# by256/icsg3d

Measured on AMD Instinct MI355X. Metric: voxel-grids/s (fwd+bwd) for 32^3 U-Net+VAE at batch 32: value = U-Net train step (BASELINE configs[1]); DFC-VAE step (configs[2]) in secondary; both per batch in unet_plus_vae, higher is better.
Workload: dtype f32

## Files before the change

icsg3d_amd/csrc/common.h:

```cpp
#pragma once
#include <hip/hip_runtime.h>
#include <hip/hip_ext.h>
#include <atomic>
#include <cstdint>
#include <cstdio>
#include <string>
#include <vector>

namespace ics {

extern std::atomic<long long> g_kernel_launches;
struct LaunchTimer {
  virtual void next(hipEvent_t* start, hipEvent_t* stop) = 0;
  virtual ~LaunchTimer() = default;
};
extern thread_local LaunchTimer* tl_launch_timer;
template <typename... P, typename... A>
inline void ics_launch(void (*kernel)(P...), dim3 grid, dim3 block, size_t shmem, hipStream_t st, A&&... args) {
  static_assert(sizeof...(P) == sizeof...(A), "kernel argument count");
  if (tl_launch_timer != nullptr) {
    hipEvent_t e0 = nullptr, e1 = nullptr;
    tl_launch_timer->next(&e0, &e1);
    hipExtLaunchKernelGGL(kernel, grid, block, (std::uint32_t)shmem, st, e0, e1, 0u, static_cast<P>(args)...);
  } else {
// ... 68 lines not shown
  CF_NO_WINO = 256,
  CF_NO_WINO_WGRAD = 512,
  CF_NO_WINO64 = 1024,
  CF_NO_UP3 = 2048,
  CF_NO_THIN1_2STAGE = 4096,
  CF_NO_FAST_BNBWD = 8192,
  CF_NO_FUSED_HEAD = 16384,
  CF_NO_BWD_FOLD = 32768,
  CF_UP3_BIG_ALWAYS = 65536,
  CF_NO_WINOG = 262144,
  CF_NO_HEAD_BNFUSE = 524288,
  CF_NO_UP3N = 1 << 21,
  CF_NO_DGRAD_BNFUSE = 1 << 22,
  CF_NO_POOL_PRESUM = 1 << 23,
  CF_NO_HEAD_LABELS = 1 << 24,
  CF_ZBATCH = 1 << 20,
};
int conv_flags_from_env();

struct ConvGeom {
  int B, S, lgS;
  int Cin, Cout;
  int taps;
  int Kpad, Npad;
  int flags = 0;
};

struct BwdStat {
  const float* s = nullptr;
  const float* mean = nullptr;
  const float* rstd = nullptr;
// ... 97 lines not shown
```

icsg3d_amd/csrc/conv_igemm.hip:

```cpp
#include "common.h"

#ifndef ICS_GEMM_DEEP_FWD_MIN
#define ICS_GEMM_DEEP_FWD_MIN 1
#endif
#ifndef ICS_GEMM_DEEP_MIN
#define ICS_GEMM_DEEP_MIN 3
#endif
#ifndef ICS_GEMM_DEEP
#define ICS_GEMM_DEEP 1
#endif

#include <algorithm>
#include <type_traits>
#include <cstdlib>
#include <cstring>
#include <vector>

namespace ics {

typedef float f32x16 __attribute__((ext_vector_type(16)));
typedef float v4f __attribute__((ext_vector_type(4)));

#ifndef ICS_KLDA
#define ICS_KLDA 36
// ... 21 lines not shown
  if (getenv("ICSG3D_NO_THIN_C")) f |= CF_NO_THIN_C;
  if (getenv("ICSG3D_NO_COND_FOLD")) f |= CF_NO_COND_FOLD;
  if (getenv("ICSG3D_NO_WINO")) f |= CF_NO_WINO;
  if (getenv("ICSG3D_NO_WINO_WGRAD")) f |= CF_NO_WINO_WGRAD;
  if (getenv("ICSG3D_NO_WINO64")) f |= CF_NO_WINO64;
  if (getenv("ICSG3D_NO_UP3")) f |= CF_NO_UP3;
  if (getenv("ICSG3D_NO_THIN1_2STAGE")) f |= CF_NO_THIN1_2STAGE;
  if (getenv("ICSG3D_NO_FAST_BNBWD")) f |= CF_NO_FAST_BNBWD;
  if (getenv("ICSG3D_NO_FUSED_HEAD")) f |= CF_NO_FUSED_HEAD;
  if (getenv("ICSG3D_NO_BWD_FOLD")) f |= CF_NO_BWD_FOLD;
  if (getenv("ICSG3D_NO_WINOG")) f |= CF_NO_WINOG;
  if (getenv("ICSG3D_NO_HEAD_BNFUSE")) f |= CF_NO_HEAD_BNFUSE;
  if (getenv("ICSG3D_NO_UP3N")) f |= CF_NO_UP3N;
  if (getenv("ICSG3D_NO_DGRAD_BNFUSE")) f |= CF_NO_DGRAD_BNFUSE;
  if (getenv("ICSG3D_NO_POOL_PRESUM")) f |= CF_NO_POOL_PRESUM;
  if (getenv("ICSG3D_NO_HEAD_LABELS")) f |= CF_NO_HEAD_LABELS;
  { const char* e = getenv("ICSG3D_UP3_BIG_MIN_WG"); if (e && *e && strtoul(e, nullptr, 10) <= 1) f |= CF_UP3_BIG_ALWAYS; }
  return f;
}
struct DevOnce {
  bool done[64] = {false};
  bool need(int* dev) {
    int d = 0;
    if (hipGetDevice(&d) != hipSuccess || d < 0 || d >= 64) { *dev = -1; return true; }
    *dev = d;
    return !done[d];
  }
  void mark(int dev) { if (dev >= 0) done[dev] = true; }
};

// ... 58 lines not shown
  r.z = act_apply(fmaf(v.z, sc.z, sh.z), slope); r.w = act_apply(fmaf(v.w, sc.w, sh.w), slope);
  return r;
}
template <bool NOACT>
__device__ __forceinline__ v4f affine_only_or_act4(v4f v, v4f sc, v4f sh, float slope) {
  if (!NOACT) return affine_act4(v, sc, sh, slope);
  v4f r;
  r.x = fmaf(v.x, sc.x, sh.x); r.y = fmaf(v.y, sc.y, sh.y); r.z = fmaf(v.z, sc.z, sh.z); r.w = fmaf(v.w, sc.w, sh.w);
  return r;
}
__device__ __forceinline__ unsigned voxel_off(int b, int z, int y, int x, int S, int u, int C) {
  const int Ss = S >> u;
  return ((((unsigned)b * Ss + (z >> u)) * Ss + (y >> u)) * Ss + (x >> u)) * (unsigned)C;
}
__device__ __forceinline__ int clampi(int v, int hi) { return min(max(v, 0), hi); }

__device__ __forceinline__ ConvSrc pick_src(const ConvSrc& s0, const ConvSrc& s1, bool first) {
  ConvSrc s;
  s.p = first ? s0.p : s1.p;
  s.scale = first ? s0.scale : s1.scale;
  s.shift = first ? s0.shift : s1.shift;
  s.C = first ? s0.C : s1.C;
  s.up = first ? s0.up : s1.up;
  s.act = first ? s0.act : s1.act;
  s.bcast = first ? s0.bcast : s1.bcast;
  return s;
}

__device__ __forceinline__ float gather_scalar(const ConvSrc& s0, const ConvSrc& s1, int ci, int b,
                                               int z, int y, int x, int S) {
// ... 225 lines not shown
      const bool kvalid = tap < g.taps;
      int dz = 0, dy = 0, dx = 0;
      if (g.taps == 27) { dz = tap / 9 - 1; dy = (tap / 3) % 3 - 1; dx = tap % 3 - 1; }
#pragma unroll
      for (int r = 0; r < RS; ++r) {
        const int m = mrow_base + 8 * r;
        const RowPos rp = decode_row(m, S, lg);
        const int zz = rp.z + dz, yy = rp.y + dy, xx = rp.x + dx;
        const bool inb = kvalid && m < M && (unsigned)zz < (unsigned)S &&
                         (unsigned)yy < (unsigned)S && (unsigned)xx < (unsigned)S;
        ras[r] = inb ? gather_scalar(s0, s1, ci, rp.b, zz, yy, xx, S) : 0.f;
      }
    }
  };

  unsigned rowG0[RA], rowG1[RA];
  if (VEC) {
#pragma unroll
    for (int r = 0; r < RA; ++r) {
      const unsigned mc = (unsigned)min(mrow_base + 32 * r, M - 1);
      rowG0[r] = (mc * (unsigned)s0.C + (unsigned)(t & 7) * 4u) * 4u;
      rowG1[r] = (mc * (unsigned)s1.C + (unsigned)(t & 7) * 4u) * 4u;
    }
  }
  auto load_chunk_gemm = [&](int c) {
    load_b(c * 8);
    const int ci0 = c << 5;
    const bool first = ci0 < s0.C;
    const int cbase = first ? ci0 : ci0 - s0.C;
    const char* sp = reinterpret_cast<const char*>(first ? s0.p : s1.p) + (size_t)cbase * 4;
    const float slope = first ? slope0 : slope1;
    v4f sc = v4f{1.f, 1.f, 1.f, 1.f}, sh = v4f{0.f, 0.f, 0.f, 0.f};
    if (AFF) {
      sc = *reinterpret_cast<const v4f*>((first ? s0.scale : s1.scale) + cbase + (t & 7) * 4);
      sh = *reinterpret_cast<const v4f*>((first ? s0.shift : s1.shift) + cbase + (t & 7) * 4);
    }
#pragma unroll
    for (int r = 0; r < RA; ++r) {
      v4f v = *reinterpret_cast<const v4f*>(sp + (first ? rowG0[r] : rowG1[r]));
      if (AFF) v = affine_only_or_act4<NOACT>(v, sc, sh, slope);
      ra4[r] = v;
    }
  };
  auto store_a_chunk = [&]() {
// ... 150 lines not shown
  const bool gemm = VEC && !THIN && !PAR && !UP && ABL == 0 && g.taps == 1;
  if (cb < ce && gemm) {
    auto compute_g = [&](int buf) { compute_at(As + (wm * TM * 32 + li) * kLDA + lh * 4, 32, buf); };
    load_chunk_gemm(cb);
    store_b(cb & 1);
    store_a_chunk();
    __syncthreads();
#if ICS_GEMM_DEEP
    if (!AFF && TM * TN >= ICS_GEMM_DEEP_FWD_MIN) {
      v4f raA[RA], rbA[NB], raB[RA], rbB[NB];
      auto load_set = [&](int c, v4f (&xa)[RA], v4f (&xb)[NB]) {
        const char* wrow = reinterpret_cast<const char*>(wp) + (size_t)(c * 8) * (size_t)g.Npad * 16;
#pragma unroll
        for (int r = 0; r < NB; ++r) xb[r] = *reinterpret_cast<const v4f*>(wrow + bofs[r]);
        const int ci0 = c << 5;
        const bool first = ci0 < s0.C;
        const char* sp = reinterpret_cast<const char*>(first ? s0.p : s1.p) + (size_t)(first ? ci0 : ci0 - s0.C) * 4;
#pragma unroll
        for (int r = 0; r < RA; ++r) xa[r] = *reinterpret_cast<const v4f*>(sp + (first ? rowG0[r] : rowG1[r]));
      };
      auto store_set = [&](int buf, const v4f (&xa)[RA], const v4f (&xb)[NB]) {
        float* Bw = Bs + buf * B_FLOATS;
#pragma unroll
        for (int r = 0; r < NB; ++r) *reinterpret_cast<v4f*>(Bw + (t + 256 * r) * 4) = xb[r];
        __syncthreads();
#pragma unroll
        for (int r = 0; r < RA; ++r) *reinterpret_cast<v4f*>(As + ((t >> 3) + 32 * r) * kLDA + (t & 7) * 4) = xa[r];
        __syncthreads();
      };
      const int lastc = ce - 1;
      if (cb + 1 < ce) load_set(cb + 1, raA, rbA);
      int c = cb;
// ... 1064 lines not shown
    return launch_conv_fwd_thin_c(st, g, src[0], g.Cin, g.Cin, wp, bias, out, ldo, pre_act, stat_partial,
                                  rows_per_block);
  ConvSrc s0 = src[0], s1 = src[nsrc > 1 ? 1 : 0];
  if (nsrc == 1) s1.C = 0;
  const bool aff = s0.scale != nullptr || (nsrc > 1 && s1.scale != nullptr);
  const bool up = s0.up || (nsrc > 1 && s1.up);
  const int variant = up ? 2 : (aff ? 1 : 0);
  const bool noact = aff && (s0.scale == nullptr || s0.act == ACT_NONE) &&
                     (nsrc < 2 || s1.scale == nullptr || s1.act == ACT_NONE);
  ICS_TRY(fix_src(s0));
  ICS_TRY(fix_src(s1));
  bool vec = fwd_is_vec(g, s0, s1);
  const bool thin = conv_is_thin(g, s0, nsrc);
  ICS_CHECK(((size_t)g.B << (3 * g.lgS)) * (size_t)std::max(s0.C, s1.C) * 4 <= 0xffffffffull,
            "conv source larger than 4 GiB");
  const bool no_reuse = (g.flags & CF_NO_REUSE) != 0;
  const bool fold = bwd != nullptr && bwd->partial != nullptr && ksplit == 1 && vec && !thin && variant == 0 &&
                    bias == nullptr && stat_partial == nullptr && !accumulate;
  int bm, bn;
  pick_fwd_tile(g, &bm, &bn);
#define ICS_FWD_ARGS st, g, s0, s1, wp, bias, out, ldo, pre_act, stat_partial, rows_per_block, accumulate, ksplit, bwd
#define ICS_FWD(WM, WN, TM, TN)                                                                 \
  do {                                                                                          \
    if (thin) return launch_fwd_cfg<WM, WN, TM, TN, true, 0, true, true, true>(ICS_FWD_ARGS);   \
    if (!vec) return launch_fwd_cfg<WM, WN, TM, TN, false, 0, true, true>(ICS_FWD_ARGS);        \
    if (g.taps == 27 && g.S >= 4 && g.S <= (WM) * (TM) * 32 && !no_reuse) {                      \
      if (variant == 0 && fold)                                                                 \
        return launch_fwd_cfg<WM, WN, TM, TN, true, 0, false, false, false, true, false, false, true>(ICS_FWD_ARGS); \
      if (variant == 0) return launch_fwd_cfg<WM, WN, TM, TN, true, 0, false, false, false, true>(ICS_FWD_ARGS); \
      if (variant == 1 && noact)                                                                \
// ... 208 lines not shown
      sc = *reinterpret_cast<const v4f*>(sv.scale + cl0);
      sh = *reinterpret_cast<const v4f*>(sv.shift + cl0);
    }
  }
  int s_tap = 0, s_ci = 0; bool s_kvalid = false; int sdz = 0, sdy = 0, sdx = 0;
  if (!VEC) {
    const int kf = k0 + (t & 31);
    s_tap = kf / g.Cin; s_ci = kf - s_tap * g.Cin; s_kvalid = kf < K;
    if (g.taps == 27) { sdz = s_tap / 9 - 1; sdy = (s_tap / 3) % 3 - 1; sdx = s_tap % 3 - 1; }
  }

  v4f ra[VEC ? APASS : 1];
  float ras[4];
  v4f rd[DPASS];

  auto load_chunk = [&](int c) {
    const int mbase = m_begin + (c << 5);
    if (VEC) {
      const int Sh = S >> 1;
#pragma unroll
      for (int p = 0; p < APASS; ++p) {
        const int m = mbase + (t + 256 * p) / AF4;
        const int x = m & (S - 1), y = (m >> lg) & (S - 1), z = (m >> (2 * lg)) & (S - 1);
        const bool inb = kvalid && m < m_end && x != xbad && y != ybad && z != zbad;
        int idx = m + sdelta;
        if (UP) {
          const int b = m >> (3 * lg);
          const int idx_up = ((b * Sh + ((z + tdz) >> 1)) * Sh + ((y + tdy) >> 1)) * Sh + ((x + tdx) >> 1);
          idx = su ? idx_up : idx;
        }
// ... 4 lines not shown
      }
    } else {
#pragma unroll
      for (int p = 0; p < 4; ++p) {
        const int m = mbase + (t >> 5) + 8 * p;
        float v = 0.f;
        if (s_kvalid && m < m_end) {
          const RowPos r = decode_row(m, S, lg);
          const int zz = r.z + sdz, yy = r.y + sdy, xx = r.x + sdx;
          if ((unsigned)zz < (unsigned)S && (unsigned)yy < (unsigned)S && (unsigned)xx < (unsigned)S)
            v = gather_scalar(s0, s1, s_ci, r.b, zz, yy, xx, S);
        }
        ras[p] = v;
      }
    }
#pragma unroll
    for (int p = 0; p < DPASS; ++p) {
      const int idx = t + 256 * p;
      const int m = mbase + idx / DF4;
      const int n = n0 + (idx % DF4) * 4;
      const float* q = dy + (size_t)min(m, M - 1) * ldy;
      v4f v;
      if (DYVEC) {
        v = *reinterpret_cast<const v4f*>(q + min(n, n_load - 4));
        if (!(m < m_end && n < n_load)) v = v4f{0.f, 0.f, 0.f, 0.f};
      } else {
        v.x = q[min(n + 0, n_load - 1)]; v.y = q[min(n + 1, n_load - 1)];
        v.z = q[min(n + 2, n_load - 1)]; v.w = q[min(n + 3, n_load - 1)];
        const bool rowok = m < m_end;
        v.x = (rowok && n + 0 < n_load) ? v.x : 0.f; v.y = (rowok && n + 1 < n_load) ? v.y : 0.f;
        v.z = (rowok && n + 2 < n_load) ? v.z : 0.f; v.w = (rowok && n + 3 < n_load) ? v.w : 0.f;
      }
      rd[p] = v;
    }
  };
  const bool gemm = VEC && DYVEC && !UP && !THIN && ABL == 0 && g.taps == 1 && (M & 31) == 0 &&
                    (rows_per_split & 31) == 0 && n0 + NT <= n_load;
  const bool noact_g = slope == 1.f;
  unsigned aoffg[VEC ? APASS : 1], doffg[DPASS];
  if (VEC) {
#pragma unroll
    for (int p = 0; p < APASS; ++p) aoffg[p] = (unsigned)(((t + 256 * p) / AF4) * sC + cl0) * 4u;
  }
#pragma unroll
  for (int p = 0; p < DPASS; ++p) {
    const int idx = t + 256 * p;
    doffg[p] = (unsigned)((idx / DF4) * ldy + n0 + (idx % DF4) * 4) * 4u;
  }
  auto load_chunk_gemm = [&](int c, auto noact_tag) {
    constexpr bool NA = decltype(noact_tag)::value;
    const int mbase = m_begin + (c << 5);
    const char* abase = reinterpret_cast<const char*>(sp) + (size_t)mbase * (size_t)sC * 4;
    const char* dbase = reinterpret_cast<const char*>(dy) + (size_t)mbase * (size_t)ldy * 4;
    if (VEC) {
#pragma unroll
      for (int p = 0; p < APASS; ++p) {
        v4f v = *reinterpret_cast<const v4f*>(abase + aoffg[p]);
        if (AFF) v = affine_only_or_act4<NA>(v, sc, sh, slope);
        ra[p] = v;
      }
    }
#pragma unroll
    for (int p = 0; p < DPASS; ++p) rd[p] = *reinterpret_cast<const v4f*>(dbase + doffg[p]);
  };
  auto store_chunk = [&](int buf) {
    float* A = As + buf * A_FLOATS;
    float* D = Ds + buf * D_FLOATS;
    if (VEC) {
// ... 56 lines not shown
        for (int j = 0; j < TN; ++j) b[j] = D[s * 2 * NT + j * 32];
      }
#pragma unroll
      for (int i = 0; i < TM; ++i)
#pragma unroll
        for (int j = 0; j < TN; ++j)
          acc[i][j] = __builtin_amdgcn_mfma_f32_32x32x2f32(a[i], b[j], acc[i][j], 0, 0, 0);
    }
  };
#if ICS_GEMM_DEEP
  if (gemm && VEC && TM * TN >= ICS_GEMM_DEEP_MIN) {
    v4f raA[APASS], rdA[DPASS], raB[APASS], rdB[DPASS];
    auto loadS = [&](int c, v4f (&xa)[APASS], v4f (&xd)[DPASS]) {
      const int mbase = m_begin + (c << 5);
      const char* abase = reinterpret_cast<const char*>(sp) + (size_t)mbase * (size_t)sC * 4;
      const char* dbase = reinterpret_cast<const char*>(dy) + (size_t)mbase * (size_t)ldy * 4;
#pragma unroll
      for (int p = 0; p < APASS; ++p) xa[p] = *reinterpret_cast<const v4f*>(abase + aoffg[p]);
#pragma unroll
      for (int p = 0; p < DPASS; ++p) xd[p] = *reinterpret_cast<const v4f*>(dbase + doffg[p]);
    };
    auto storeS = [&](int buf, const v4f (&xa)[APASS], const v4f (&xd)[DPASS]) {
      float* A = As + buf * A_FLOATS;
      float* D = Ds + buf * D_FLOATS;
#pragma unroll
      for (int p = 0; p < APASS; ++p) {
        const int idx = t + 256 * p;
        v4f v = xa[p];
        if (AFF) v = noact_g ? affine_only_or_act4<true>(v, sc, sh, slope) : affine_only_or_act4<false>(v, sc, sh, slope);
        *reinterpret_cast<v4f*>(A + (idx / AF4) * KT + (idx % AF4) * 4) = v;
      }
// ... 623 lines not shown
#undef ICS_TNW
      ICS_HIP(hipGetLastError());
    }
    if (phase != 1)
      ICS_TRY(launch_reduce_splits(st, workspace, (M + rows - 1) / rows, n_el, g.Cout, dw, ldw, sub_rows, row_pitch,
                                   row_off));
    return 0;
  }
  ConvSrc s0 = src[0], s1 = src[nsrc > 1 ? 1 : 0];
  if (nsrc == 1) s1.C = 0;
  ICS_TRY(fix_src(s0));
  ICS_TRY(fix_src(s1));
  WgradPlan p = plan_wgrad(g, s0, nsrc, s1);
  const size_t n_elems = (size_t)g.taps * g.Cin * g.Cout;
  const int n_load4 = (g.Cout + 3) / 4 * 4;
  const bool dy_vec = (ldy % 4 == 0) && ((reinterpret_cast<uintptr_t>(dy) & 15) == 0) && (n_load4 <= ldy);
  const int n_load = dy_vec ? n_load4 : g.Cout;
  if (!dy_vec) {
    p.nt = (p.kt == 128) ? 32 : (p.kt == 64) ? 64 : 128;
    p.ntiles = (g.Npad + p.nt - 1) / p.nt;
  }
  const bool aff = src[0].scale != nullptr || (nsrc > 1 && src[1].scale != nullptr);
  const bool up = src[0].up || (nsrc > 1 && src[1].up);
  if (dy_vec && wgrad3_ok(g, s0, nsrc, s1)) {
    const Wgrad3Plan q = plan_wgrad3(g);
    ICS_CHECK((size_t)q.ksplit * n_elems <= workspace_floats, "wgrad workspace too small");
    const int arows = 32 + std::max(32 >> g.lgS, 1) + 1;
    const size_t lds = (size_t)(2 * (arows * 64 + 32 * 128) + 128) * sizeof(float);
    const dim3 grid(9 * q.cgroups * q.ntiles * q.ksplit);
    const int M3 = g.B << (3 * g.lgS);
    const bool fast = !up && g.lgS >= 4 && g.lgS <= 6 && M3 % 32 == 0 && n_load == g.Cout &&
// ... 444 lines not shown
```

icsg3d_amd/csrc/elementwise.h:

```cpp
#pragma once
#include "common.h"

#include <rccl/rccl.h>

namespace ics {

struct BnParams {
  const float* gamma;
  const float* beta;
  float* moving_mean;
  float* moving_var;
  float* mean;
  float* rstd;
  float* scale;
  float* shift;
  float* xs = nullptr;
};

struct BnSync {
  ncclComm_t comm;
  int nranks;
  double* local;
  double* gathered;
};
// ... 92 lines not shown
                    const float* cond, int ncond, int B, float* z, float* zc);
int launch_vae_loss(hipStream_t st, const float* mulv, int ld, int latent, int B, const double* mse_partial,
                    int n_mse, double n_elems, const double* pm_partial, const PmSums& pmc, float alpha, float beta,
                    float* metrics, double* sums = nullptr, int phase = 0);
int launch_vae_dz(hipStream_t st, const float* mulv, int ld, int latent, int B, const float* eps,
                  const float* dzc, int ldzc, float beta, float* dmulv);
int launch_cond_bias_table(hipStream_t st, const float* w, const float* bias, const float* cond, int C, int ncond,
                           int Cin_tot, int Cout, int B, float* T);
size_t cond_wgrad_workspace_doubles(int B, int Cout);
int launch_cond_wgrad(hipStream_t st, const float* dy, int B, int S, int Cout, const float* cond, int C0, int nfold,
                      int ncond, int Cin_tot, float* dw, double* ws, size_t ws_doubles);
int launch_relu_bwd(hipStream_t st, const float* a, float* g, size_t n);
int launch_colsum_small(hipStream_t st, const float* a, int rows, int cols, int ld, float* out);
int launch_axpy(hipStream_t st, float* y, const float* x, size_t n, float a);
int launch_pool27(hipStream_t st, const float* dy, int B, int S, int N, float* out, int ldo);
int launch_permute_up_dw(hipStream_t st, const float* tmp, int Cu, int N, int Cin, int c_off, float* dw);

}
```

icsg3d_amd/csrc/elementwise.hip:

```cpp
#include "common.h"
#include "elementwise.h"

namespace ics {

__device__ __forceinline__ double wave_sum_d(double v) {
#pragma unroll
  for (int o = 32; o > 0; o >>= 1) v += __shfl_xor(v, o);
  return v;
}
__device__ __forceinline__ float wave_sum_f(float v) {
#pragma unroll
  for (int o = 32; o > 0; o >>= 1) v += __shfl_xor(v, o);
  return v;
}
__device__ __forceinline__ float wave_max_f(float v) {
#pragma unroll
  for (int o = 32; o > 0; o >>= 1) v = fmaxf(v, __shfl_xor(v, o));
  return v;
}
__device__ __forceinline__ double block_sum_d(double v, double* sh ) {
  v = wave_sum_d(v);
  __syncthreads();
  if ((threadIdx.x & 63) == 0) sh[threadIdx.x >> 6] = v;
  __syncthreads();
// ... 1741 lines not shown
        if (sz <= 1) o[2 * 9 + dyi * 3 + dx] += P[dyi][dx];
        if (sz >= 1 && sz <= 2) o[1 * 9 + dyi * 3 + dx] += P[dyi][dx];
        if (sz >= 2) o[0 * 9 + dyi * 3 + dx] += P[dyi][dx];
      }
  }
#pragma unroll
  for (int k = 0; k < 27; ++k) *reinterpret_cast<pf4*>(out + vl * ldo + (size_t)k * N + n) = o[k];
}
int launch_pool27(hipStream_t st, const float* dy, int B, int S, int N, float* out, int ldo) {
  ICS_CHECK(N % 4 == 0 && ldo % 4 == 0, "pool27: channel counts must be multiples of 4");
  const size_t total = (size_t)B * (S / 2) * (S / 2) * (S / 2) * (N / 4);
  ICS_LAUNCH(pool27_kernel, dim3((unsigned)((total + 255) / 256)), dim3(256), 0, st, dy, B, S, N, total, out, ldo);
  ICS_HIP(hipGetLastError());
  return 0;
}
__global__ void permute_up_dw_kernel(const float* __restrict__ tmp, int Cu, int N, int Cin, int c_off,
                                     size_t total, float* __restrict__ dw) {
  const size_t i = (size_t)blockIdx.x * blockDim.x + threadIdx.x;
  if (i >= total) return;
  const int n = (int)(i % N);
  size_t r = i / N;
  const int c = (int)(r % Cu);
  const int tap = (int)(r / Cu);
  dw[((size_t)tap * Cin + c_off + c) * N + n] = tmp[(size_t)c * 27 * N + (size_t)tap * N + n];
}
int launch_permute_up_dw(hipStream_t st, const float* tmp, int Cu, int N, int Cin, int c_off, float* dw) {
  const size_t total = (size_t)27 * Cu * N;
  ICS_LAUNCH(permute_up_dw_kernel, dim3((unsigned)((total + 255) / 256)), dim3(256), 0, st, tmp, Cu, N, Cin,
                     c_off, total, dw);
  ICS_HIP(hipGetLastError());
// ... 324 lines not shown
```

icsg3d_amd/csrc/engine.hip:

```cpp
#include "common.h"
#include "elementwise.h"
#include "segment.h"
#include "scratch.h"
#include "voxelise.h"
#include "latent.h"
#include "tsne.h"
#include "render.h"
#include "monitor.h"
#include "../../include/icsg3d.h"

#include <rccl/rccl.h>
#include <roctracer/roctx.h>

#include <cmath>
#include <cstring>
#include <map>
#include <memory>
#include <mutex>
#include <vector>

namespace ics {

struct Range {
  explicit Range(const char* name) { roctxRangePushA(name); }
// ... 130 lines not shown
  ConvLayer* skip_prod = nullptr;
  ConvLayer* deferred_skip = nullptr;
  float* pooled = nullptr;
  unsigned char* pool_idx = nullptr;
  ConvSrc src[2];
  int nsrc = 1;
  bool split_up = false;
  bool wf_stale = false;
  int Cs = 0, Cu = 0;
  float *wf_skip = nullptr, *w_up = nullptr;
  float *wp_skip = nullptr, *wp_par = nullptr;
  float* w_up3 = nullptr;
  float* w_up3n = nullptr;
  float *dyS = nullptr;
  int ldS = 0;
  float *dA_skip = nullptr, *dxl = nullptr;
  float *dw_up = nullptr;
};

struct Net {
  int kind = 0;
  int device = 0;
  int flags = 0;
  hipStream_t st = nullptr;
  hipStream_t st2 = nullptr;
  hipEvent_t ev_fork = nullptr, ev_join = nullptr;
  bool side_on = true, side_dirty = false;
  bool pm_side = false;
  int maxB = 0, d = 0, C = 0;
  std::vector<void*> allocs;
// ... 257 lines not shown
}

static ConvSrc src_plain(const float* p, int C) { return ConvSrc{p, nullptr, nullptr, C, 0, ACT_NONE, 0}; }
static ConvSrc src_layer(const ConvLayer& L, int up) {
  if (L.has_bn) return ConvSrc{L.s, L.scale, L.shift, L.Cout, up, L.post_act, 0};
  return ConvSrc{L.s, nullptr, nullptr, L.Cout, up, ACT_NONE, 0};
}

static ConvGeom geom_fwd(const ConvLayer& L, int B) {
  return ConvGeom{B, L.S, ilog2(L.S), L.CinG, L.Cout, L.taps, L.Kpad, L.Npad, L.flags};
}
static ConvGeom geom_bwd(const ConvLayer& L, int B) {
  return ConvGeom{B, L.S, ilog2(L.S), L.Cout, L.CinG, L.taps, L.Kpad_b, L.Npad_b, L.flags};
}

static ConvGeom geom_up_wgrad(const ConvLayer& L, int B) {
  return ConvGeom{B, L.S / 2, ilog2(L.S / 2), L.Cu, 27 * L.Cout, 1, round_up(L.Cu, 32), L.ldS, L.flags};
}
static ConvGeom geom_up_dgrad(const ConvLayer& L, int B) {
  return ConvGeom{B, L.S / 2, ilog2(L.S / 2), L.ldS, L.Cu, 1, L.ldS, round_up(L.Cu, 32), L.flags};
}
static ConvGeom geom_skip_wgrad(const ConvLayer& L, int B) {
  return ConvGeom{B, L.S, ilog2(L.S), L.Cs, L.Cout, L.taps, round_up(L.taps * L.Cs, 32), L.Npad, L.flags};
}
static ConvGeom geom_skip_dgrad(const ConvLayer& L, int B) {
  return ConvGeom{B, L.S, ilog2(L.S), L.Cout, L.Cs, L.taps, L.Kpad_b, round_up(L.Cs, 32), L.flags};
}
static ConvGeom geom_skip_fwd(const ConvLayer& L, int B) {
  return ConvGeom{B, L.S, ilog2(L.S), L.Cs, L.Cout, L.taps, round_up(L.taps * L.Cs, 32), L.Npad, L.flags};
}
static ConvGeom geom_par_fwd(const ConvLayer& L, int B) {
  return ConvGeom{B, L.S / 2, ilog2(L.S / 2), L.Cu, L.Cout, 8, 8 * L.Cu, L.Npad, L.flags};
}
static ConvSrc src_lowres(const ConvLayer& L) { ConvSrc u = L.src[L.nsrc - 1]; u.up = 0; return u; }

static int enable_split_up(Net& n, ConvLayer& L) {
  if (n.flags & CF_NO_UPSPLIT) return 0;
  const ConvSrc& up = L.src[L.nsrc - 1];
  const int Cs = L.nsrc == 2 ? L.src[0].C : 0;
  if (!up.up || (L.nsrc == 2 && L.src[0].up) || L.taps != 27 || L.S < 2 || L.CinG != L.Cin || Cs % 32 || up.C % 32 ||
      up.bcast || L.Cout % 4)
    return 0;
  L.split_up = true;
  L.Cs = Cs; L.Cu = up.C;
  L.ldS = round_up(27 * L.Cout, 32);
  const size_t M = n.rows(L, n.maxB);
  ICS_TRY(n.alloc(&L.w_up, (size_t)L.ldS * round_up(L.Cu, 32)));
  ICS_TRY(n.alloc(&L.dyS, M / 8 * L.ldS));
  ICS_HIP(hipMemsetAsync(L.dyS, 0, M / 8 * L.ldS * sizeof(float), n.st));
  ICS_TRY(n.alloc(&L.dxl, M / 8 * L.Cu));
  ICS_TRY(n.alloc(&L.dw_up, (size_t)L.Cu * 27 * L.Cout));
  if (conv_up3_ok(geom_par_fwd(L, n.maxB), src_lowres(L)))
    ICS_TRY(n.alloc(&L.w_up3, conv_up3_weight_floats(L.Cu, L.Cout)));
  else if (L.Cs == 0 && conv_up3n_ok(geom_par_fwd(L, n.maxB), src_lowres(L)))
    ICS_TRY(n.alloc(&L.w_up3n, conv_up3n_weight_floats(L.Cu, L.Cout)));
  else
    ICS_TRY(n.alloc(&L.wp_par, (size_t)8 * 8 * L.Cu * L.Npad));
  if (L.Cs) {
    ICS_TRY(n.alloc(&L.wf_skip, (size_t)L.Kpad_b * round_up(L.Cs, 32)));
    ICS_TRY(n.alloc(&L.dA_skip, M * L.Cs));
    ICS_TRY(n.alloc(&L.wp_skip, (size_t)round_up(L.taps * L.Cs, 32) * L.Npad));
  }
  return 0;
}
// ... 47 lines not shown
static int alloc_workspaces(Net& n, bool need_bwd) {
  size_t stat = 0, bwd = 0, wg = 0, fw = 0;
  for (int b = 1; b <= n.maxB; ++b)
  for (auto& Lp : n.layers) {
    ConvLayer& L = *Lp;
    const size_t M = n.rows(L, b);
    const ConvGeom g = geom_fwd(L, b);
    const int rpb = std::min(conv_fwd_rows_per_block(g), 64);
    stat = std::max(stat, (M + rpb - 1) / rpb * 3 * (size_t)L.Npad);
    if (L.split_up) stat = std::max(stat, 8 * ((M / 8 + 63) / 64) * 3 * (size_t)L.Npad);
    fw = std::max(fw, conv_fwd_workspace_floats(g, L.src, L.nsrc));
    if (need_bwd) {
      const ConvSrc sdy = src_plain(L.dy, L.Cout);
      fw = std::max(fw, conv_fwd_workspace_floats(geom_bwd(L, b), &sdy, 1));
      if (L.split_up) {
        const ConvSrc sd = src_plain(L.dyS, L.ldS);
        fw = std::max(fw, conv_fwd_workspace_floats(geom_up_dgrad(L, b), &sd, 1));
        if (L.Cs) fw = std::max(fw, conv_fwd_workspace_floats(geom_skip_dgrad(L, b), &sdy, 1));
      }
      LayerBwd lb{};
      lb.B = b; lb.S = L.S; lb.lgS = ilog2(L.S); lb.C = L.Cout;
      if (&L != n.head) bwd = std::max(bwd, layer_bwd_workspace_floats(lb));
      wg = std::max(wg, conv_wgrad_workspace_floats(g, L.src, L.nsrc));
      if (L.wino_w)
        wg = std::max(wg, conv_wino_wgrad_workspace_floats(L.split_up ? geom_skip_wgrad(L, b) : g));
      if ((L.Cin == 1 || L.cond_fold) && (L.Cout == 16 || L.Cout == 32))
        wg = std::max(wg, conv_thin_c_wgrad_workspace_floats(g));
      if (L.split_up) {
        const ConvSrc lo = src_lowres(L);
        wg = std::max(wg, conv_wgrad_workspace_floats(geom_up_wgrad(L, b), &lo, 1));
        if (L.Cs) wg = std::max(wg, conv_wgrad_workspace_floats(geom_skip_wgrad(L, b), L.src, 1));
// ... 247 lines not shown
      L.src[0].act != ACT_NONE || !n.want_wgrad_inputs || P->tie_batch != B)
    return false;
  if (!L.wino_w || !L.wwb || L.wwb_layout != 1) return false;
  if (n.rows(L, B) * (size_t)P->Cout * sizeof(float) < 2 * n.bnfuse_min_bytes) return false;
  const ConvGeom gw = geom_skip_wgrad(L, B), gd = geom_skip_dgrad(L, B);
  const ConvSrc sdy = src_plain(L.dy, L.Cout);
  return conv_bnfuse_ok(L.S, L.Cs, L.Cout) && conv_wino_wgrad_ok(gw, L.src, 1) && conv_wino_ok(gd, &sdy, 1) &&
         conv_bnfuse_partial_floats(B, L.S, L.Cout) <= n.ws_cls_n && L.Cs % 4 == 0 &&
         pool_bnfuse_partial_doubles(n.rows(L, B) / 8, P->Cout) <= n.ws_pool_n;
}
static int conv_grads_split_up(Net& n, ConvLayer& L, int B, ConvLayer* next) {
  const size_t M = n.rows(L, B);
  const double fl_skip = 2.0 * M * 27 * L.Cs * L.Cout, fl_up = 2.0 * (M / 8) * 27 * L.Cu * L.Cout;
  const bool skipfuse = skip_bnfuse_ok(n, L, B);
  ConvLayer* P = L.skip_prod;
  n.prof.begin(n.st, "pool27:" + L.name, 0, 4.0 * M * L.Cout * (1 + 27.0 / 8));
  ICS_TRY(launch_pool27(n.st, L.dy, B, L.S, L.Cout, L.dyS, L.ldS));
  n.prof.end(n.st);
  hipStream_t ws = side_begin(n);
  if (L.Cs) {
    const ConvGeom g = geom_skip_wgrad(L, B);
    n.prof.begin(ws, "conv_wgrad:" + L.name + ".skip|", fl_skip,
                 4.0 * (M * L.Cs + M * L.Cout + 27.0 * L.Cs * L.Cout));
    const bool wino = L.wino_w && conv_wino_wgrad_ok(g, L.src, 1);
    ConvSrc sx = L.src[0];
    if (skipfuse) { sx.scale = P->xs; sx.shift = P->xs + P->Cout; }
    if (wino)
      ICS_TRY(launch_conv_wgrad_wino(ws, g, sx, L.dy, L.Cout, n.tg(L.t_w), L.Cout, n.ws_wgrad, n.ws_wgrad_n,
                                     L.Cs, L.Cin, 0, 1));
    else
    ICS_TRY(launch_conv_wgrad(ws, g, L.src, 1, L.dy, L.Cout, n.tg(L.t_w), L.Cout, n.ws_wgrad, n.ws_wgrad_n, L.Cs,
                              L.Cin, 0, 1));
    n.prof.end(ws);
// ... 8 lines not shown
    if (skipfuse) {
      const bool pend = L.db_blocks > 0;
      n.prof.begin(ws, "bnfuse:" + L.name + ".skip", 0, 0);
      ICS_TRY(launch_conv_bnfuse(ws, L.dy, B, L.S, L.Cs, L.Cin, L.Cout, pend ? L.db_partial : n.tg(L.t_b), pend ? L.db_blocks : 1,
                                 n.tp(L.t_w), n.tg(L.t_w), n.tp(P->t_gamma), n.tp(P->t_beta), P->mean, P->rstd, P->scale,
                                 nullptr, nullptr, nullptr, nullptr, n.ws_cls, n.ws_cls_n, n.ws_R, P->bn_sums));
      n.prof.end(ws);
      P->deferred_skip = &L;
    }
  }
  {
    const ConvGeom g = geom_up_wgrad(L, B);
    const ConvSrc lo = src_lowres(L);
    n.prof.begin(ws, "conv_wgrad:" + L.name + ".up|", fl_up,
                 4.0 * (M / 8 * L.Cu + M / 8 * 27.0 * L.Cout + 27.0 * L.Cu * L.Cout));
    ICS_TRY(launch_conv_wgrad(ws, g, &lo, 1, L.dyS, L.ldS, L.dw_up, 27 * L.Cout, n.ws_wgrad, n.ws_wgrad_n, 0, 0, 0, 1));
    n.prof.end(ws);
    n.prof.begin(ws, "wgrad_reduce_splits", 0, 0);
    ICS_TRY(launch_conv_wgrad(ws, g, &lo, 1, L.dyS, L.ldS, L.dw_up, 27 * L.Cout, n.ws_wgrad, n.ws_wgrad_n, 0, 0, 0, 2));
    ICS_TRY(launch_permute_up_dw(ws, L.dw_up, L.Cu, L.Cout, L.Cin, L.Cs, n.tg(L.t_w)));
    n.prof.end(ws);
  }
  if (L.Cs && !skipfuse) {
    const ConvGeom g = geom_skip_dgrad(L, B);
    ConvSrc sdy = src_plain(L.dy, L.Cout);
    n.prof.begin(n.st, "conv_dgrad:" + L.name + ".skip|", fl_skip,
                 4.0 * (M * L.Cs + M * L.Cout + 27.0 * L.Cs * L.Cout));
    if (L.wwb && conv_wino_ok(g, &sdy, 1))
      ICS_TRY(launch_conv_fwd_wino(n.st, g, sdy, L.wwb, nullptr, L.dA_skip, L.Cs, ACT_NONE, nullptr, nullptr, 0,
                                   L.wwb_layout));
    else
    ICS_TRY(launch_conv_fwd(n.st, g, &sdy, 1, L.wf_skip, nullptr, L.dA_skip, L.Cs, ACT_NONE, nullptr, nullptr, 0,
                            n.fws(), n.ws_fwd_n));
    n.prof.end(n.st);
  }
  {
    const ConvGeom g = geom_up_dgrad(L, B);
    ConvSrc sd = src_plain(L.dyS, L.ldS);
    n.prof.begin(n.st, "conv_dgrad:" + L.name + ".up|", fl_up,
                 4.0 * (M / 8 * L.Cu + M / 8 * 27.0 * L.Cout + 27.0 * L.Cu * L.Cout));
    const BwdStat bs = bwd_stat_for(n, next, B);
    int blocks = 0;
    ICS_TRY(launch_conv_fwd(n.st, g, &sd, 1, L.w_up, nullptr, L.dxl, L.Cu, ACT_NONE, nullptr, nullptr, 0, n.fws(),
                            n.ws_fwd_n, &bs, &blocks));
    bwd_stat_done(next, bs, blocks, g.Npad);
    n.prof.end(n.st);
  }
  return 0;
}

static int colsum_push(Net& n, const float* partial, int nblk, int C, float* out);
static bool dgrad_bnfuse_ok(const Net& n, const ConvLayer& L, const ConvLayer* next, int B, bool need_dA, bool param_grads) {
  if (next == nullptr || !need_dA || !param_grads || (n.flags & CF_NO_DGRAD_BNFUSE) || n.sync() != nullptr || n.side_on)
// ... 2111 lines not shown
        for (int z = 0; z < h; ++z)
          for (int y = 0; y < h; ++y)
            for (int x = 0; x < h; ++x) {
              float* o = s.dx + ((((size_t)b * h + z) * h + y) * h + x) * s.C;
              for (int c = 0; c < s.C; ++c) o[c] = 0.f;
              for (int k = 0; k < 8; ++k) {
                const size_t m = (((size_t)b * S + 2 * z + (k >> 2)) * S + 2 * y + ((k >> 1) & 1)) * S + 2 * x + (k & 1);
                for (int c = 0; c < s.C; ++c) o[c] += hA[m * ld + c0 + c];
              }
            }
    }
  }
  if (a->kernels && a->kernels_cap > 0) {
    std::string txt;
    for (const auto& r : n.prof.rows)
      if (r.label.find('|') != std::string::npos) txt += r.label + "\n";
    std::strncpy(a->kernels, txt.c_str(), (size_t)a->kernels_cap - 1);
    a->kernels[a->kernels_cap - 1] = 0;
  }
  if (n.canary_on) {
    std::string msg;
    const int bad = n.canaries_dirty(&msg);
    ICS_CHECK(bad == 0, op + "guard bytes written behind " + std::to_string(bad) + " buffer(s): " + msg);
  }
  return 0;
}

int ics_op_conv_link(ics_conv_link* a) {
  const std::string op = "ics_op_conv_link: ";
  ICS_CHECK(a != nullptr, op + "null argument");
  ICS_CHECK(a->link >= ICS_LINK_SAME && a->link <= ICS_LINK_POOL_SKIP, op + "unknown link");
// ... 309 lines not shown
```

icsg3d_amd/engine.py:

```python
from __future__ import annotations

import ctypes as C

import numpy as np

from . import _lib as L


def _f32(a):
    return np.ascontiguousarray(a, dtype=np.float32)


def _jobs4(jobs):
    jobs = np.ascontiguousarray(jobs, np.int32)
    if jobs.ndim != 2 or jobs.shape[1] != 4:
        raise ValueError("jobs must be (B, 4) int32 {structure, r0, r1, r2}, got %s" % (jobs.shape,))
    return jobs


class _Net:

    def __init__(self):
        self._h = L._H(None)
        self._lib = L.load()
# ... 538 lines not shown
            setattr(a, k, L.fptr(r[k]))
    if dout is not None:
        r["dw"], r["dbias"] = out(w.shape), out((Cout,))
        a.dw, a.dbias = L.fptr(r["dw"]), L.fptr(r["dbias"])
        if has_bn:
            r["dgamma"], r["dbeta"] = out((Cout,)), out((Cout,))
            a.dgamma, a.dbeta = L.fptr(r["dgamma"]), L.fptr(r["dbeta"])
        r["dx"] = dxs
    text = C.create_string_buffer(16384)
    a.kernels, a.kernels_cap = C.cast(text, C.c_void_p), len(text)
    L.check(lib.ics_op_conv_layer(C.byref(a)))
    if has_bn:
        r["rows_per_block"], r["blocks"] = a.rows_per_block, a.blocks
    lines = text.value.decode().splitlines()
    r["kernels"] = {k: [ln for ln in lines if ln.startswith("conv_%s:" % k)] for k in ("fwd", "dgrad", "wgrad")}
    return r


LINKS = ("same", "up", "pool", "pool_skip")


def conv_link(link, x0, layers, dout, form="unet", q=None, dout_l=None, pool_ties_all=True, max_batch=None):
    lib = L.load()
    a = L.ConvLinkArgs()
    keep = []

    def f(v):
        if v is None:
            return None
        v = _f32(v)
# ... 65 lines not shown
```

Measured before the change: 1147.

## Replace 27-tap pooled up-split operand with 8-phase pooled volume and gathered addressing

The backward of split upsampling layers used to build a pooled operand with 27 tap slabs per low-res voxel (pool27). It now builds a smaller 8-phase pooled volume on a padded (S/2+1)^3 grid (pool8). The implicit-GEMM dgrad and wgrad kernels address it through a new CF_GATHER8 mode that maps each tap to a phase and row offset. This reduces the bytes written and read for the pooled dy, at the cost of extra index arithmetic in the inner load loops and less regular access.

```diff
diff --git a/icsg3d_amd/csrc/common.h b/icsg3d_amd/csrc/common.h
--- a/icsg3d_amd/csrc/common.h
+++ b/icsg3d_amd/csrc/common.h
@@ -106,7 +106,9 @@
   CF_NO_DGRAD_BNFUSE = 1 << 22,
   CF_NO_POOL_PRESUM = 1 << 23,
   CF_NO_HEAD_LABELS = 1 << 24,
+  CF_NO_POOL8 = 1 << 25,
   CF_ZBATCH = 1 << 20,
+  CF_GATHER8 = 1 << 26,
 };
 int conv_flags_from_env();
 
diff --git a/icsg3d_amd/csrc/conv_igemm.hip b/icsg3d_amd/csrc/conv_igemm.hip
--- a/icsg3d_amd/csrc/conv_igemm.hip
+++ b/icsg3d_amd/csrc/conv_igemm.hip
@@ -59,6 +59,7 @@
   if (getenv("ICSG3D_NO_UP3N")) f |= CF_NO_UP3N;
   if (getenv("ICSG3D_NO_DGRAD_BNFUSE")) f |= CF_NO_DGRAD_BNFUSE;
   if (getenv("ICSG3D_NO_POOL_PRESUM")) f |= CF_NO_POOL_PRESUM;
+  if (getenv("ICSG3D_NO_POOL8")) f |= CF_NO_POOL8;
   if (getenv("ICSG3D_NO_HEAD_LABELS")) f |= CF_NO_HEAD_LABELS;
   { const char* e = getenv("ICSG3D_UP3_BIG_MIN_WG"); if (e && *e && strtoul(e, nullptr, 10) <= 1) f |= CF_UP3_BIG_ALWAYS; }
   return f;
@@ -147,6 +148,21 @@
   return ((((unsigned)b * Ss + (z >> u)) * Ss + (y >> u)) * Ss + (x >> u)) * (unsigned)C;
 }
 __device__ __forceinline__ int clampi(int v, int hi) { return min(max(v, 0), hi); }
+
+__device__ __forceinline__ int rowq_lin(int m, int S, int lg) {
+  const int P = S + 1;
+  const int x = m & (S - 1), y = (m >> lg) & (S - 1), z = (m >> (2 * lg)) & (S - 1), b = m >> (3 * lg);
+  return ((b * P + z) * P + y) * P + x;
+}
+__device__ __forceinline__ unsigned gather8_rcp(int N) { return 0xffffffffu / (unsigned)N + 1u; }
+__device__ __forceinline__ unsigned gather8_off(int k, int N, unsigned rcpN, int S, int ld) {
+  const int P = S + 1;
+  const int tap = (int)__umulhi((unsigned)k, rcpN), n = k - tap * N;
+  const int kz = tap / 9, ky = (tap / 3) % 3, kx = tap % 3;
+  const int roff = (((kz != 2) * P + (ky != 2)) * P + (kx != 2));
+  const int ph = 4 * (kz != 1) + 2 * (ky != 1) + (kx != 1);
+  return (unsigned)(roff * ld + ph * N + n);
+}
 
 __device__ __forceinline__ ConvSrc pick_src(const ConvSrc& s0, const ConvSrc& s1, bool first) {
   ConvSrc s;
@@ -402,11 +418,15 @@
     }
   };
 
+  const bool g8 = (g.flags & CF_GATHER8) != 0;
+  const int g8N = g8 ? g.Cin / 27 : 2;
+  const unsigned g8R = gather8_rcp(g8N);
   unsigned rowG0[RA], rowG1[RA];
   if (VEC) {
 #pragma unroll
     for (int r = 0; r < RA; ++r) {
-      const unsigned mc = (unsigned)min(mrow_base + 32 * r, M - 1);
+      unsigned mc = (unsigned)min(mrow_base + 32 * r, M - 1);
+      if (g8) mc = (unsigned)rowq_lin((int)mc, S, lg);
       rowG0[r] = (mc * (unsigned)s0.C + (unsigned)(t & 7) * 4u) * 4u;
       rowG1[r] = (mc * (unsigned)s1.C + (unsigned)(t & 7) * 4u) * 4u;
     }
@@ -414,8 +434,8 @@
   auto load_chunk_gemm = [&](int c) {
     load_b(c * 8);
     const int ci0 = c << 5;
-    const bool first = ci0 < s0.C;
-    const int cbase = first ? ci0 : ci0 - s0.C;
+    const bool first = g8 || ci0 < s0.C;
+    const int cbase = g8 ? (int)gather8_off(ci0, g8N, g8R, S, s0.C) : (first ? ci0 : ci0 - s0.C);
     const char* sp = reinterpret_cast<const char*>(first ? s0.p : s1.p) + (size_t)cbase * 4;
     const float slope = first ? slope0 : slope1;
     v4f sc = v4f{1.f, 1.f, 1.f, 1.f}, sh = v4f{0.f, 0.f, 0.f, 0.f};
@@ -596,8 +616,9 @@
 #pragma unroll
         for (int r = 0; r < NB; ++r) xb[r] = *reinterpret_cast<const v4f*>(wrow + bofs[r]);
         const int ci0 = c << 5;
-        const bool first = ci0 < s0.C;
-        const char* sp = reinterpret_cast<const char*>(first ? s0.p : s1.p) + (size_t)(first ? ci0 : ci0 - s0.C) * 4;
+        const bool first = g8 || ci0 < s0.C;
+        const int cbase = g8 ? (int)gather8_off(ci0, g8N, g8R, S, s0.C) : (first ? ci0 : ci0 - s0.C);
+        const char* sp = reinterpret_cast<const char*>(first ? s0.p : s1.p) + (size_t)cbase * 4;
 #pragma unroll
         for (int r = 0; r < RA; ++r) xa[r] = *reinterpret_cast<const v4f*>(sp + (first ? rowG0[r] : rowG1[r]));
       };
@@ -1692,6 +1713,13 @@
   const bool thin = conv_is_thin(g, s0, nsrc);
   ICS_CHECK(((size_t)g.B << (3 * g.lgS)) * (size_t)std::max(s0.C, s1.C) * 4 <= 0xffffffffull,
             "conv source larger than 4 GiB");
+  if (g.flags & CF_GATHER8) {
+    const size_t P = (size_t)g.S + 1;
+    ICS_CHECK(g.taps == 1 && nsrc == 1 && vec && !thin && variant == 0 && g.Cin % (27 * 32) == 0 && g.Kpad == g.Cin &&
+                  src[0].C >= 8 * (g.Cin / 27),
+              "gathered up-split operand: plain source, 27 tap slabs of N % 32 == 0 columns");
+    ICS_CHECK((size_t)g.B * P * P * P * (size_t)s0.C * 4 <= 0xffffffffull, "phase volumes larger than 4 GiB");
+  }
   const bool no_reuse = (g.flags & CF_NO_REUSE) != 0;
   const bool fold = bwd != nullptr && bwd->partial != nullptr && ksplit == 1 && vec && !thin && variant == 0 &&
                     bias == nullptr && stat_partial == nullptr && !accumulate;
@@ -1930,6 +1958,14 @@
   float ras[4];
   v4f rd[DPASS];
 
+  const bool g8 = DYVEC && (g.flags & CF_GATHER8) != 0;
+  unsigned gq[DPASS];
+#pragma unroll
+  for (int p = 0; p < DPASS; ++p) {
+    const int nc = max(min(n0 + ((t + 256 * p) % DF4) * 4, n_load - 4), 0);
+    gq[p] = g8 ? gather8_off(nc, g.Cout / 27, gather8_rcp(g.Cout / 27), S, ldy) : 0u;
+  }
+
   auto load_chunk = [&](int c) {
     const int mbase = m_begin + (c << 5);
     if (VEC) {
@@ -1964,25 +2000,30 @@
         ras[p] = v;
       }
     }
-#pragma unroll
-    for (int p = 0; p < DPASS; ++p) {
-      const int idx = t + 256 * p;
-      const int m = mbase + idx / DF4;
-      const int n = n0 + (idx % DF4) * 4;
-      const float* q = dy + (size_t)min(m, M - 1) * ldy;
-      v4f v;
-      if (DYVEC) {
-        v = *reinterpret_cast<const v4f*>(q + min(n, n_load - 4));
-        if (!(m < m_end && n < n_load)) v = v4f{0.f, 0.f, 0.f, 0.f};
-      } else {
-        v.x = q[min(n + 0, n_load - 1)]; v.y = q[min(n + 1, n_load - 1)];
-        v.z = q[min(n + 2, n_load - 1)]; v.w = q[min(n + 3, n_load - 1)];
-        const bool rowok = m < m_end;
-        v.x = (rowok && n + 0 < n_load) ? v.x : 0.f; v.y = (rowok && n + 1 < n_load) ? v.y : 0.f;
-        v.z = (rowok && n + 2 < n_load) ? v.z : 0.f; v.w = (rowok && n + 3 < n_load) ? v.w : 0.f;
-      }
-      rd[p] = v;
-    }
+    auto load_d = [&](auto gather_tag) {
+      constexpr bool G8 = decltype(gather_tag)::value;
+#pragma unroll
+      for (int p = 0; p < DPASS; ++p) {
+        const int idx = t + 256 * p;
+        const int m = mbase + idx / DF4;
+        const int n = n0 + (idx % DF4) * 4;
+        const int mc = min(m, M - 1);
+        const float* q = dy + (size_t)(G8 ? rowq_lin(mc, S, lg) : mc) * ldy;
+        v4f v;
+        if (DYVEC) {
+          v = *reinterpret_cast<const v4f*>(q + (G8 ? (int)gq[p] : min(n, n_load - 4)));
+          if (!(m < m_end && n < n_load)) v = v4f{0.f, 0.f, 0.f, 0.f};
+        } else {
+          v.x = q[min(n + 0, n_load - 1)]; v.y = q[min(n + 1, n_load - 1)];
+          v.z = q[min(n + 2, n_load - 1)]; v.w = q[min(n + 3, n_load - 1)];
+          const bool rowok = m < m_end;
+          v.x = (rowok && n + 0 < n_load) ? v.x : 0.f; v.y = (rowok && n + 1 < n_load) ? v.y : 0.f;
+          v.z = (rowok && n + 2 < n_load) ? v.z : 0.f; v.w = (rowok && n + 3 < n_load) ? v.w : 0.f;
+        }
+        rd[p] = v;
+      }
+    };
+    if (g8) load_d(std::true_type{}); else load_d(std::false_type{});
   };
   const bool gemm = VEC && DYVEC && !UP && !THIN && ABL == 0 && g.taps == 1 && (M & 31) == 0 &&
                     (rows_per_split & 31) == 0 && n0 + NT <= n_load;
@@ -1995,13 +2036,14 @@
 #pragma unroll
   for (int p = 0; p < DPASS; ++p) {
     const int idx = t + 256 * p;
-    doffg[p] = (unsigned)((idx / DF4) * ldy + n0 + (idx % DF4) * 4) * 4u;
+    doffg[p] = g8 ? (unsigned)(rowq_lin(idx / DF4, S, lg) * ldy + (int)gq[p]) * 4u
+                  : (unsigned)((idx / DF4) * ldy + n0 + (idx % DF4) * 4) * 4u;
   }
   auto load_chunk_gemm = [&](int c, auto noact_tag) {
     constexpr bool NA = decltype(noact_tag)::value;
     const int mbase = m_begin + (c << 5);
     const char* abase = reinterpret_cast<const char*>(sp) + (size_t)mbase * (size_t)sC * 4;
-    const char* dbase = reinterpret_cast<const char*>(dy) + (size_t)mbase * (size_t)ldy * 4;
+    const char* dbase = reinterpret_cast<const char*>(dy) + (size_t)(g8 ? rowq_lin(mbase, S, lg) : mbase) * (size_t)ldy * 4;
     if (VEC) {
 #pragma unroll
       for (int p = 0; p < APASS; ++p) {
@@ -2088,7 +2130,7 @@
     auto loadS = [&](int c, v4f (&xa)[APASS], v4f (&xd)[DPASS]) {
       const int mbase = m_begin + (c << 5);
       const char* abase = reinterpret_cast<const char*>(sp) + (size_t)mbase * (size_t)sC * 4;
-      const char* dbase = reinterpret_cast<const char*>(dy) + (size_t)mbase * (size_t)ldy * 4;
+      const char* dbase = reinterpret_cast<const char*>(dy) + (size_t)(g8 ? rowq_lin(mbase, S, lg) : mbase) * (size_t)ldy * 4;
 #pragma unroll
       for (int p = 0; p < APASS; ++p) xa[p] = *reinterpret_cast<const v4f*>(abase + aoffg[p]);
 #pragma unroll
@@ -2742,7 +2784,15 @@
   WgradPlan p = plan_wgrad(g, s0, nsrc, s1);
   const size_t n_elems = (size_t)g.taps * g.Cin * g.Cout;
   const int n_load4 = (g.Cout + 3) / 4 * 4;
-  const bool dy_vec = (ldy % 4 == 0) && ((reinterpret_cast<uintptr_t>(dy) & 15) == 0) && (n_load4 <= ldy);
+  const bool gather8 = (g.flags & CF_GATHER8) != 0;
+  if (gather8) {
+    const size_t P = (size_t)g.S + 1;
+    ICS_CHECK(g.taps == 1 && g.Cout % (27 * 4) == 0 && ldy >= 8 * (g.Cout / 27) && ldy % 4 == 0 &&
+                  (reinterpret_cast<uintptr_t>(dy) & 15) == 0 && !wgrad3_ok(g, s0, nsrc, s1),
+              "gathered up-split operand: 27 tap slabs of N % 4 == 0 columns");
+    ICS_CHECK((size_t)g.B * P * P * P * (size_t)ldy * 4 <= 0xffffffffull, "phase volumes larger than 4 GiB");
+  }
+  const bool dy_vec = (ldy % 4 == 0) && ((reinterpret_cast<uintptr_t>(dy) & 15) == 0) && (gather8 || n_load4 <= ldy);
   const int n_load = dy_vec ? n_load4 : g.Cout;
   if (!dy_vec) {
     p.nt = (p.kt == 128) ? 32 : (p.kt == 64) ? 64 : 128;
diff --git a/icsg3d_amd/csrc/elementwise.h b/icsg3d_amd/csrc/elementwise.h
--- a/icsg3d_amd/csrc/elementwise.h
+++ b/icsg3d_amd/csrc/elementwise.h
@@ -130,6 +130,7 @@
 int launch_colsum_small(hipStream_t st, const float* a, int rows, int cols, int ld, float* out);
 int launch_axpy(hipStream_t st, float* y, const float* x, size_t n, float a);
 int launch_pool27(hipStream_t st, const float* dy, int B, int S, int N, float* out, int ldo);
+int launch_pool8(hipStream_t st, const float* dy, int B, int S, int N, float* out, int ldo);
 int launch_permute_up_dw(hipStream_t st, const float* tmp, int Cu, int N, int Cin, int c_off, float* dw);
 
 }
diff --git a/icsg3d_amd/csrc/elementwise.hip b/icsg3d_amd/csrc/elementwise.hip
--- a/icsg3d_amd/csrc/elementwise.hip
+++ b/icsg3d_amd/csrc/elementwise.hip
@@ -1779,6 +1779,60 @@
   ICS_HIP(hipGetLastError());
   return 0;
 }
+__global__ __launch_bounds__(256) void pool8_kernel(const float* __restrict__ dy, int B, int S, int N, size_t total,
+                                                    float* __restrict__ out, int ldo) {
+  const size_t i = (size_t)blockIdx.x * blockDim.x + threadIdx.x;
+  if (i >= total) return;
+  const int P = (S >> 1) + 1, N4 = N >> 2;
+  const int n = (int)(i % N4) * 4;
+  const size_t row = i / N4;
+  const int ix = row % P; size_t r = row / P;
+  const int iy = r % P; r /= P;
+  const int iz = r % P;
+  const int b = (int)(r / P);
+  const pf4 zero = pf4{0.f, 0.f, 0.f, 0.f};
+  pf4 o[8];
+#pragma unroll
+  for (int k = 0; k < 8; ++k) o[k] = zero;
+#pragma unroll
+  for (int sz = 0; sz < 3; ++sz) {
+    const int z = 2 * iz - 2 + sz;
+    if ((unsigned)z >= (unsigned)S) continue;
+    pf4 lx[3][2];
+#pragma unroll
+    for (int sy = 0; sy < 3; ++sy) {
+      const int y = 2 * iy - 2 + sy;
+      pf4 v[3];
+#pragma unroll
+      for (int sx = 0; sx < 3; ++sx) {
+        const int x = 2 * ix - 2 + sx;
+        const bool ok = (unsigned)y < (unsigned)S && (unsigned)x < (unsigned)S;
+        v[sx] = ok ? *reinterpret_cast<const pf4*>(dy + ((((size_t)b * S + z) * S + y) * S + x) * N + n) : zero;
+      }
+      lx[sy][0] = v[0] + v[1];
+      lx[sy][1] = v[1] + v[2];
+    }
+#pragma unroll
+    for (int oy = 0; oy < 2; ++oy)
+#pragma unroll
+      for (int ox = 0; ox < 2; ++ox) {
+        const pf4 p = lx[oy][ox] + lx[oy + 1][ox];
+        if (sz <= 1) o[2 * oy + ox] += p;
+        if (sz >= 1) o[4 + 2 * oy + ox] += p;
+      }
+  }
+#pragma unroll
+  for (int k = 0; k < 8; ++k) *reinterpret_cast<pf4*>(out + row * ldo + (size_t)k * N + n) = o[k];
+}
+int launch_pool8(hipStream_t st, const float* dy, int B, int S, int N, float* out, int ldo) {
+  ICS_CHECK(N % 4 == 0 && ldo % 4 == 0 && ldo >= 8 * N, "pool8: channel counts must be multiples of 4");
+  const size_t P = (size_t)S / 2 + 1;
+  const size_t total = (size_t)B * P * P * P * (N / 4);
+  ICS_CHECK((total + 255) / 256 <= 0x7fffffffull, "pool8: grid too large");
+  ICS_LAUNCH(pool8_kernel, dim3((unsigned)((total + 255) / 256)), dim3(256), 0, st, dy, B, S, N, total, out, ldo);
+  ICS_HIP(hipGetLastError());
+  return 0;
+}
 __global__ void permute_up_dw_kernel(const float* __restrict__ tmp, int Cu, int N, int Cin, int c_off,
                                      size_t total, float* __restrict__ dw) {
   const size_t i = (size_t)blockIdx.x * blockDim.x + threadIdx.x;
diff --git a/icsg3d_amd/csrc/engine.hip b/icsg3d_amd/csrc/engine.hip
--- a/icsg3d_amd/csrc/engine.hip
+++ b/icsg3d_amd/csrc/engine.hip
@@ -168,6 +168,9 @@
   float* w_up3n = nullptr;
   float *dyS = nullptr;
   int ldS = 0;
+  bool pool8 = false;
+  float* Q = nullptr;
+  int ldQ = 0;
   float *dA_skip = nullptr, *dxl = nullptr;
   float *dw_up = nullptr;
 };
@@ -455,12 +458,14 @@
   return ConvGeom{B, L.S, ilog2(L.S), L.Cout, L.CinG, L.taps, L.Kpad_b, L.Npad_b, L.flags};
 }
 
+static int up_flags(const ConvLayer& L) { return L.pool8 ? (L.flags | CF_GATHER8) : L.flags; }
 static ConvGeom geom_up_wgrad(const ConvLayer& L, int B) {
-  return ConvGeom{B, L.S / 2, ilog2(L.S / 2), L.Cu, 27 * L.Cout, 1, round_up(L.Cu, 32), L.ldS, L.flags};
+  return ConvGeom{B, L.S / 2, ilog2(L.S / 2), L.Cu, 27 * L.Cout, 1, round_up(L.Cu, 32), L.ldS, up_flags(L)};
 }
 static ConvGeom geom_up_dgrad(const ConvLayer& L, int B) {
-  return ConvGeom{B, L.S / 2, ilog2(L.S / 2), L.ldS, L.Cu, 1, L.ldS, round_up(L.Cu, 32), L.flags};
-}
+  return ConvGeom{B, L.S / 2, ilog2(L.S / 2), L.ldS, L.Cu, 1, L.ldS, round_up(L.Cu, 32), up_flags(L)};
+}
+static ConvSrc src_up_pooled(const ConvLayer& L) { return L.pool8 ? src_plain(L.Q, L.ldQ) : src_plain(L.dyS, L.ldS); }
 static ConvGeom geom_skip_wgrad(const ConvLayer& L, int B) {
   return ConvGeom{B, L.S, ilog2(L.S), L.Cs, L.Cout, L.taps, round_up(L.taps * L.Cs, 32), L.Npad, L.flags};
 }
@@ -487,8 +492,16 @@
   L.ldS = round_up(27 * L.Cout, 32);
   const size_t M = n.rows(L, n.maxB);
   ICS_TRY(n.alloc(&L.w_up, (size_t)L.ldS * round_up(L.Cu, 32)));
-  ICS_TRY(n.alloc(&L.dyS, M / 8 * L.ldS));
-  ICS_HIP(hipMemsetAsync(L.dyS, 0, M / 8 * L.ldS * sizeof(float), n.st));
+  const size_t Pq = (size_t)L.S / 2 + 1, rowsQ = (size_t)n.maxB * Pq * Pq * Pq;
+  L.pool8 = !(n.flags & CF_NO_POOL8) && L.Cout % 32 == 0 && rowsQ * 8 * L.Cout * sizeof(float) <= 0xffffffffull;
+  if (L.pool8) {
+    L.ldQ = 8 * L.Cout;
+    ICS_TRY(n.alloc(&L.Q, rowsQ * L.ldQ));
+    ICS_HIP(hipMemsetAsync(L.Q, 0, rowsQ * L.ldQ * sizeof(float), n.st));
+  } else {
+    ICS_TRY(n.alloc(&L.dyS, M / 8 * L.ldS));
+    ICS_HIP(hipMemsetAsync(L.dyS, 0, M / 8 * L.ldS * sizeof(float), n.st));
+  }
   ICS_TRY(n.alloc(&L.dxl, M / 8 * L.Cu));
   ICS_TRY(n.alloc(&L.dw_up, (size_t)L.Cu * 27 * L.Cout));
   if (conv_up3_ok(geom_par_fwd(L, n.maxB), src_lowres(L)))
@@ -566,7 +579,7 @@
       const ConvSrc sdy = src_plain(L.dy, L.Cout);
       fw = std::max(fw, conv_fwd_workspace_floats(geom_bwd(L, b), &sdy, 1));
       if (L.split_up) {
-        const ConvSrc sd = src_plain(L.dyS, L.ldS);
+        const ConvSrc sd = src_up_pooled(L);
         fw = std::max(fw, conv_fwd_workspace_floats(geom_up_dgrad(L, b), &sd, 1));
         if (L.Cs) fw = std::max(fw, conv_fwd_workspace_floats(geom_skip_dgrad(L, b), &sdy, 1));
       }
@@ -844,9 +857,17 @@
   const double fl_skip = 2.0 * M * 27 * L.Cs * L.Cout, fl_up = 2.0 * (M / 8) * 27 * L.Cu * L.Cout;
   const bool skipfuse = skip_bnfuse_ok(n, L, B);
   ConvLayer* P = L.skip_prod;
-  n.prof.begin(n.st, "pool27:" + L.name, 0, 4.0 * M * L.Cout * (1 + 27.0 / 8));
-  ICS_TRY(launch_pool27(n.st, L.dy, B, L.S, L.Cout, L.dyS, L.ldS));
+  if (L.pool8) {
+    const double Pq = L.S / 2 + 1;
+    n.prof.begin(n.st, "pool8:" + L.name, 0, 4.0 * L.Cout * (M + 8.0 * B * Pq * Pq * Pq));
+    ICS_TRY(launch_pool8(n.st, L.dy, B, L.S, L.Cout, L.Q, L.ldQ));
+  } else {
+    n.prof.begin(n.st, "pool27:" + L.name, 0, 4.0 * M * L.Cout * (1 + 27.0 / 8));
+    ICS_TRY(launch_pool27(n.st, L.dy, B, L.S, L.Cout, L.dyS, L.ldS));
+  }
   n.prof.end(n.st);
+  const float* pooled = L.pool8 ? L.Q : L.dyS;
+  const int ld_pooled = L.pool8 ? L.ldQ : L.ldS;
   hipStream_t ws = side_begin(n);
   if (L.Cs) {
     const ConvGeom g = geom_skip_wgrad(L, B);
@@ -885,10 +906,10 @@
     const ConvSrc lo = src_lowres(L);
     n.prof.begin(ws, "conv_wgrad:" + L.name + ".up|", fl_up,
                  4.0 * (M / 8 * L.Cu + M / 8 * 27.0 * L.Cout + 27.0 * L.Cu * L.Cout));
-    ICS_TRY(launch_conv_wgrad(ws, g, &lo, 1, L.dyS, L.ldS, L.dw_up, 27 * L.Cout, n.ws_wgrad, n.ws_wgrad_n, 0, 0, 0, 1));
+    ICS_TRY(launch_conv_wgrad(ws, g, &lo, 1, pooled, ld_pooled, L.dw_up, 27 * L.Cout, n.ws_wgrad, n.ws_wgrad_n, 0, 0, 0, 1));
     n.prof.end(ws);
     n.prof.begin(ws, "wgrad_reduce_splits", 0, 0);
-    ICS_TRY(launch_conv_wgrad(ws, g, &lo, 1, L.dyS, L.ldS, L.dw_up, 27 * L.Cout, n.ws_wgrad, n.ws_wgrad_n, 0, 0, 0, 2));
+    ICS_TRY(launch_conv_wgrad(ws, g, &lo, 1, pooled, ld_pooled, L.dw_up, 27 * L.Cout, n.ws_wgrad, n.ws_wgrad_n, 0, 0, 0, 2));
     ICS_TRY(launch_permute_up_dw(ws, L.dw_up, L.Cu, L.Cout, L.Cin, L.Cs, n.tg(L.t_w)));
     n.prof.end(ws);
   }
@@ -907,7 +928,7 @@
   }
   {
     const ConvGeom g = geom_up_dgrad(L, B);
-    ConvSrc sd = src_plain(L.dyS, L.ldS);
+    ConvSrc sd = src_up_pooled(L);
     n.prof.begin(n.st, "conv_dgrad:" + L.name + ".up|", fl_up,
                  4.0 * (M / 8 * L.Cu + M / 8 * 27.0 * L.Cout + 27.0 * L.Cu * L.Cout));
     const BwdStat bs = bwd_stat_for(n, next, B);
@@ -3049,7 +3070,7 @@
   if (a->kernels && a->kernels_cap > 0) {
     std::string txt;
     for (const auto& r : n.prof.rows)
-      if (r.label.find('|') != std::string::npos) txt += r.label + "\n";
+      txt += r.label + "\n";
     std::strncpy(a->kernels, txt.c_str(), (size_t)a->kernels_cap - 1);
     a->kernels[a->kernels_cap - 1] = 0;
   }
diff --git a/icsg3d_amd/engine.py b/icsg3d_amd/engine.py
--- a/icsg3d_amd/engine.py
+++ b/icsg3d_amd/engine.py
@@ -576,6 +576,7 @@
         r["rows_per_block"], r["blocks"] = a.rows_per_block, a.blocks
     lines = text.value.decode().splitlines()
     r["kernels"] = {k: [ln for ln in lines if ln.startswith("conv_%s:" % k)] for k in ("fwd", "dgrad", "wgrad")}
+    r["sites"] = lines
     return r
 
 
```

New measurement: 1156, median of 6. No clear change (+0.8%).
